# dohlee/chromoformer

Measured on AMD Instinct MI355X. Metric: genes/sec training (bsz=64, default config), higher is better.
Workload: dtype f32

## Files before the change

### chromoformer_amd/csrc/cf_attc2.h

```cpp
#pragma once
#include <type_traits>

namespace cf {

struct Attc2Args {
    const float* feats[kMaxRes];
    const uint8_t* mask[kMaxRes];
    long long mstride[kMaxRes];
    const float* pe[kMaxRes];
    const float* pet[kMaxRes];
    const float* wlp[kMaxRes];
    const float* vin[kMaxRes];
    float* p[kMaxRes];
    float* w[kMaxRes];
    float* vout[kMaxRes];
    int L[kMaxRes], Lpad[kMaxRes], LT[kMaxRes];
    int N, F;
    float scale, rscale;
    unsigned long long* tdbg;
    unsigned long long* tall;
};
#define CF_STAMP2(slot)                                                                                   \
    do {                                                                                                  \
        if (a.tdbg && stamp_wg == 0 && (threadIdx.x & 63) == 0)                                            \
// ... 9 lines not shown

__device__ __forceinline__ void frag_load_nn_rt(FragNN<4, 8>& f, const float* __restrict__ Bm, int ldb, int nchunks) {
    const int lane = threadIdx.x & 63, r = lane & 15, q = lane >> 4;
    f.bp = Bm + (size_t)(q * 4) * ldb + 4 * r;
    f.ldb = ldb;
#pragma unroll
    for (int c = 0; c < kRing - 1; ++c) frag_chunk_nn(f, c, min(c, nchunks - 1));
    __builtin_amdgcn_sched_barrier(0);
}
__device__ __forceinline__ void frag_mma_nn_rt(FragNN<4, 8>& f, const float* As, int lda, int nchunks, f32x4 (&acc)[4]) {
    const int lane = threadIdx.x & 63, r = lane & 15, q = lane >> 4;
    const float* ap = As + r * lda + q * 4;
    float4 a_nxt = *reinterpret_cast<const float4*>(ap);
    for (int c0 = 0; c0 < nchunks; c0 += kRing) {
#pragma unroll
        for (int u = 0; u < kRing; ++u) {
            const int c = c0 + u;
            if (c + kRing - 1 < nchunks) frag_chunk_nn(f, (u + kRing - 1) % kRing, c + kRing - 1);
            __builtin_amdgcn_sched_barrier(0);
            if (c < nchunks)
#pragma unroll
                for (int k = 0; k < 2; ++k) {
                    const float4 a = a_nxt;
                    a_nxt = *reinterpret_cast<const float4*>(ap + (c * 2 + k + 1) * 16);
                    const float av[4] = {a.x, a.y, a.z, a.w};
#pragma unroll
                    for (int i = 0; i < 4; ++i) {
                        const float* bv = reinterpret_cast<const float*>(&f.ring[u][k][i]);
#pragma unroll
                        for (int t = 0; t < 4; ++t) acc[t] = mfma4(av[i], bv[t], acc[t]);
                    }
                }
        }
    }
}

__host__ __device__ inline size_t attc2_scratch_floats(int L) { return (size_t)kTile * (attc2_lpad(L) + 4) + 2 * kTile * (kD + 4) + 2 * kTile * 8; }
__host__ __device__ inline size_t attc2_persist_bytes(int L, int F, int AG) {
    return (size_t)(kD * 8 + AG * L * F + 8) * sizeof(float) + (size_t)AG * attc2_lpad(L);
}
template <int AG>
__device__ __forceinline__ void attc2_stage(const float* feats, const uint8_t* mask, long long mstride, const float* wlp, int L, int Lpad, int F,
                                            const int n0, const int N, float* persist) {
    const int tid = threadIdx.x, w = __builtin_amdgcn_readfirstlane(tid >> 6);
    float* wlp_s = persist;
    float* feats_s = wlp_s + kD * 8;
    uint8_t* mk_s = reinterpret_cast<uint8_t*>(feats_s + AG * L * F + 8);
    const int nreg = min(AG, N - n0);
    const float* fg = feats + (size_t)n0 * L * F;
    const int nf = nreg * L * F;
    constexpr int NFL = AG == 8 ? 12 : AG == 4 ? 6 : AG == 2 ? 3 : 2;
    const bool f16b = ((L * F) & 3) == 0 && AG * L * F <= NFL * 4 * kAT && (reinterpret_cast<uintptr_t>(fg) & 15) == 0;
    if (f16b) {
        const int n4 = (AG * L * F) >> 2, last4 = (nf >> 2) - 1;
#pragma unroll
        for (int u = 0; u < NFL; ++u) {
            const int i = tid + u * kAT;
            typedef __attribute__((address_space(3))) void* lds_void;
            typedef const __attribute__((address_space(1))) void* glb_void;
            if (i < n4)
                __builtin_amdgcn_global_load_lds((glb_void)(fg + (size_t)min(i, last4) * 4), (lds_void)(feats_s + (size_t)(w * 64 + u * kAT) * 4), 16, 0, 0);
        }
    } else {
        for (int i = tid; i < AG * L * F; i += kAT) feats_s[i] = i < nf ? ldg(fg + i) : 0.f;
    }
    if (tid < 8) feats_s[AG * L * F + tid] = 0.f;
    static_assert(kD * 8 == 2 * kAT, "wlp staging assumes two entries per thread");
    wlp_s[tid] = (tid & 7) < F ? ldg(wlp + (tid >> 3) * F + (tid & 7)) : 0.f;
    wlp_s[tid + kAT] = (tid & 7) < F ? ldg(wlp + ((tid + kAT) >> 3) * F + (tid & 7)) : 0.f;
    const uint8_t* mg = mask + (size_t)n0 * mstride;
    const bool words = ((L | (int)mstride | (int)(reinterpret_cast<uintptr_t>(mask))) & 3) == 0;
    if (words) {
        const int LW = Lpad >> 2, lw = L >> 2;
        uint32_t* mk_w = reinterpret_cast<uint32_t*>(mk_s);
        for (int idx = tid; idx < AG * LW; idx += kAT) {
            const int sreg = idx / LW, jw = idx - sreg * LW;
            mk_w[idx] = (sreg < nreg && jw < lw) ? *(const CF_GLOBAL uint32_t*)(mg + (size_t)sreg * mstride + 4 * jw) : 0x01010101u;
        }
    } else {
        for (int s = 0; s < AG; ++s)
            for (int j = tid; j < Lpad; j += kAT) mk_s[s * Lpad + j] = (s < nreg && j < L) ? *(const CF_GLOBAL uint8_t*)(mg + (size_t)s * mstride + j) : (uint8_t)1;
    }
}
template <bool BWD, int AG, bool STAGED = false>
__device__ __forceinline__ void attc2_body(const Attc2Args& a, const int r, const int n0, const int N, float* scratch, float* persist,
                                           const int stamp_wg = -1) {
    constexpr int kAG = AG;
    const int tid = threadIdx.x;
    const int w = tid >> 6, lane = tid & 63, lr = lane & 15, lq = lane >> 4;
    const int L = a.L[r], Lpad = a.Lpad[r], LT = a.LT[r], F = a.F, LS = Lpad + 4;
    constexpr int LD = kD + 4, NW = kAT / 64;
    float* sc_s = scratch;
    float* vin_s = sc_s + kTile * LS;
    float* red_s = vin_s + kTile * LD;
    float* u_s = red_s + kTile * LD;
    float* w_s = u_s + kTile * 8;
    float* wlp_s = persist;
    float* feats_s = wlp_s + kD * 8;
    uint8_t* mk_s = reinterpret_cast<uint8_t*>(feats_s + kAG * L * F + 8);
    const int nreg = min(kAG, N - n0);

    CF_STAMP2(0);
    if (a.tall && tid == 0 && stamp_wg >= 0) a.tall[stamp_wg * 2] = __builtin_amdgcn_s_memtime();
    const int nblk = (L + 63) / 64;
    float* stat_s = red_s;
    static_assert(2 * kTile * 16 <= kTile * LD, "statistics fit in the K-split partial buffer");
    FragNN<4, 8> ft0;
    const float* fg = a.feats[r] + (size_t)n0 * L * F;
    const int nf = nreg * L * F;
    constexpr int NFL = AG == 8 ? 12 : AG == 4 ? 6 : AG == 2 ? 3 : 2;
    const bool f16b = ((L * F) & 3) == 0 && kAG * L * F <= NFL * 4 * kAT;
    float4 fv12[NFL];
    {
        const uint8_t* mg = a.mask[r] + (size_t)n0 * a.mstride[r];
        const bool words = ((L | (int)a.mstride[r] | (int)(reinterpret_cast<uintptr_t>(a.mask[r]))) & 3) == 0;
        const int LW = Lpad >> 2, lw = L >> 2;
        constexpr int MW = kAG >= 2 ? kAG / 2 : 1;
        float4 vv = make_float4(0.f, 0.f, 0.f, 0.f);
        {
            const int m = tid >> 5, c4 = tid & 31;
            if ((m >> 1) < nreg) vv = ldg4(a.vin[r] + (size_t)n0 * 256 + m * kD + c4 * 4);
        }
        const float wl0 = !STAGED && (tid & 7) < F ? ldg(a.wlp[r] + (tid >> 3) * F + (tid & 7)) : 0.f;
        const float wl1 = !STAGED && (tid & 7) < F ? ldg(a.wlp[r] + ((tid + kAT) >> 3) * F + (tid & 7)) : 0.f;
        uint32_t mwv[MW];
        if (!STAGED && words) {
#pragma unroll
            for (int k = 0; k < MW; ++k) {
                const int idx = tid + k * kAT, sreg = idx / LW, jw = idx - sreg * LW;
                mwv[k] = (idx < kAG * LW && sreg < nreg && jw < lw) ? *(const CF_GLOBAL uint32_t*)(mg + (size_t)sreg * a.mstride[r] + 4 * jw) : 0x01010101u;
            }
        }
        {
            if (!STAGED) {
                const float* fa = reinterpret_cast<const float*>(reinterpret_cast<uintptr_t>(fg) & ~(uintptr_t)15);
                const int last4 = f16b ? (nf >> 2) - 1 : max((nf >> 2) - 2, 0);
#pragma unroll
                for (int u = 0; u < NFL; ++u) fv12[u] = ldg4(fa + (size_t)min(tid + u * kAT, last4) * 4);
            }
            const float* bm_ = a.pet[r] + min(w, nblk - 1) * 64;
            ft0.bp = bm_ + (size_t)(lq * 4) * LT + 4 * lr;
            ft0.ldb = LT;
            frag_chunk_nn(ft0, 0, 0);
        }
        __builtin_amdgcn_sched_barrier(0);
        stat_s[tid] = tid < kTile * 16 ? 0.f : -INFINITY;
        if (tid < kTile) u_s[tid * 8 + 7] = 0.f;
        {
            const int m = tid >> 5;
            for (int j = L + (tid & 31); j < Lpad; j += 32) sc_s[m * LS + j] = 0.f;
        }
        *reinterpret_cast<float4*>(vin_s + (tid >> 5) * LD + (tid & 31) * 4) = vv;
        static_assert(kD * 8 == 2 * kAT, "wlp staging assumes two entries per thread");
        if (!STAGED) {
            wlp_s[tid] = wl0;
            wlp_s[tid + kAT] = wl1;
        }
        if (STAGED) {
        } else if (words) {
            uint32_t* mk_w = reinterpret_cast<uint32_t*>(mk_s);
#pragma unroll
            for (int k = 0; k < MW; ++k)
                if (tid + k * kAT < kAG * LW) mk_w[tid + k * kAT] = mwv[k];
        } else {
            for (int s = 0; s < kAG; ++s)
                for (int j = tid; j < Lpad; j += kAT)
                    mk_s[s * Lpad + j] = (s < nreg && j < L) ? *(const CF_GLOBAL uint8_t*)(mg + (size_t)s * a.mstride[r] + j) : (uint8_t)1;
        }
    }
    CF_STAMP2(10);
    __syncthreads();
    CF_STAMP2(1);
    float ub[32];
    if (w == NW - 1) {
        const float* wp_ = a.wlp[r] + (size_t)(lq * 4) * F + min(lr, F - 1);
#pragma unroll
        for (int st8 = 0; st8 < 8; ++st8)
#pragma unroll
            for (int i = 0; i < 4; ++i) ub[st8 * 4 + i] = ldg(wp_ + (size_t)(st8 * 16 + i) * F);
    }
    f32x4 acc2[2][4];
    zero_acc(acc2[0]);
    zero_acc(acc2[1]);
    {
        const float* ap = vin_s + lr * LD + lq * 4;
        auto products = [&](auto c_c) {
            constexpr int c = decltype(c_c)::value;
            if (w < nblk)
#pragma unroll
                for (int k = 0; k < 2; ++k) {
                    const float4 av4 = *reinterpret_cast<const float4*>(ap + (c * 2 + k) * 16);
                    const float av[4] = {av4.x, av4.y, av4.z, av4.w};
#pragma unroll
                    for (int i = 0; i < 4; ++i) {
                        const float* bv = reinterpret_cast<const float*>(&ft0.ring[c][k][i]);
#pragma unroll
                        for (int t = 0; t < 4; ++t) acc2[0][t] = mfma4(av[i], bv[t], acc2[0][t]);
                    }
                }
        };
        frag_chunk_nn(ft0, 1, 1);
        frag_chunk_nn(ft0, 2, 2);
        __builtin_amdgcn_sched_barrier(0);
        if (w == NW - 1) {
            f32x4 ua = {0.f, 0.f, 0.f, 0.f};
#pragma unroll
            for (int st8 = 0; st8 < 8; ++st8) {
                const float4 av = *reinterpret_cast<const float4*>(ap + st8 * 16);
                ua = mfma4(av.x, ub[st8 * 4], ua);
                ua = mfma4(av.y, ub[st8 * 4 + 1], ua);
                ua = mfma4(av.z, ub[st8 * 4 + 2], ua);
                ua = mfma4(av.w, ub[st8 * 4 + 3], ua);
            }
            if (lr < F)
#pragma unroll
                for (int ii = 0; ii < 4; ++ii) u_s[(lq * 4 + ii) * 8 + lr] = ua[ii];
        }
        __builtin_amdgcn_sched_barrier(0);
        products(std::integral_constant<int, 0>{});
        __builtin_amdgcn_sched_barrier(0);
        frag_chunk_nn(ft0, 3, 3);
        __builtin_amdgcn_sched_barrier(0);
        products(std::integral_constant<int, 1>{});
        products(std::integral_constant<int, 2>{});
        products(std::integral_constant<int, 3>{});
    }
    if (w + NW < nblk) {
        FragNN<4, 8> ft;
        frag_load_nn(ft, a.pet[r] + (w + NW) * 64, LT);
        frag_mma_nn(ft, vin_s, LD, acc2[1]);
    }
    CF_STAMP2(8);
    if (STAGED) {
    } else if (f16b) {
        const int n4 = (kAG * L * F) >> 2;
#pragma unroll
        for (int u = 0; u < NFL; ++u) {
            const int i = tid + u * kAT;
            if (i < n4) *reinterpret_cast<float4*>(feats_s + (size_t)i * 4) = fv12[u];
        }
        if (tid < 8) feats_s[kAG * L * F + tid] = 0.f;
    } else {
        for (int i = tid; i < kAG * L * F + 8; i += kAT) feats_s[i] = i < nf ? ldg(fg + i) : 0.f;
    }
    const int cg = w & 1, kh = w >> 1, kper = Lpad / 4;
    FragNN<4, 8> fp5;
    frag_load_nn_rt(fp5, a.pe[r] + (size_t)(kh * kper) * kD + cg * 64, kD, kper / 32);
    CF_STAMP2(9);
    __syncthreads();
    CF_STAMP2(2);
    float xs[2][4][4];
    float4 pv[2][4];
    float bstat[2][4];
#pragma unroll
    for (int bi = 0; bi < 2; ++bi) {
        const int jb = w + bi * NW;
        if (jb >= nblk) continue;
        const int j0 = jb * 64 + 4 * lr;
        if (BWD) {
#pragma unroll
            for (int ii = 0; ii < 4; ++ii) {
                const int m = lq * 4 + ii;
                pv[bi][ii] = make_float4(0.f, 0.f, 0.f, 0.f);
                if ((m >> 1) < nreg && (m >> 1) < kAG) {
                    const float* pg = a.p[r] + ((size_t)n0 * 2 + m) * L;
                    if (j0 + 3 < L && (L & 3) == 0) pv[bi][ii] = (CF_TRUNK_NT & 2) ? ldg4_nt(pg + j0) : ldg4(pg + j0);
                    else {
                        if (j0 < L) pv[bi][ii].x = ldg(pg + j0);
                        if (j0 + 1 < L) pv[bi][ii].y = ldg(pg + j0 + 1);
                        if (j0 + 2 < L) pv[bi][ii].z = ldg(pg + j0 + 2);
                        if (j0 + 3 < L) pv[bi][ii].w = ldg(pg + j0 + 3);
                    }
                }
            }
        }
#pragma unroll
        for (int sp = 0; sp < 2; ++sp) {
            const int s = lq * 2 + sp;
            if (s >= kAG) continue;
            float fv[4][8];
            if (j0 + 3 < L && F == 7) {
                const float4* fp4 = reinterpret_cast<const float4*>(feats_s + (size_t)(s * L + j0) * 7);
                float tmp[28];
#pragma unroll
                for (int k = 0; k < 7; ++k) {
                    const float4 t4 = fp4[k];
                    tmp[4 * k] = t4.x;
                    tmp[4 * k + 1] = t4.y;
                    tmp[4 * k + 2] = t4.z;
                    tmp[4 * k + 3] = t4.w;
                }
#pragma unroll
                for (int t = 0; t < 4; ++t)
#pragma unroll
                    for (int f = 0; f < 8; ++f) fv[t][f] = f < 7 ? tmp[t * 7 + f] : 0.f;
            } else {
#pragma unroll
                for (int t = 0; t < 4; ++t)
#pragma unroll
                    for (int f = 0; f < 8; ++f) fv[t][f] = (j0 + t < L && f < F) ? feats_s[(size_t)(s * L + j0 + t) * F + f] : 0.f;
            }
            const uint32_t mw = *reinterpret_cast<const uint32_t*>(mk_s + s * Lpad + j0);
#pragma unroll
            for (int hd = 0; hd < 2; ++hd) {
                const int ii = sp * 2 + hd, m = lq * 4 + ii;
                const float4 u0 = *reinterpret_cast<const float4*>(u_s + m * 8), u1 = *reinterpret_cast<const float4*>(u_s + m * 8 + 4);
                float bm = -INFINITY;
#pragma unroll
                for (int t = 0; t < 4; ++t) {
                    float x = acc2[bi][t][ii];
                    x = fmaf(fv[t][0], u0.x, x);
                    x = fmaf(fv[t][1], u0.y, x);
                    x = fmaf(fv[t][2], u0.z, x);
                    x = fmaf(fv[t][3], u0.w, x);
                    x = fmaf(fv[t][4], u1.x, x);
                    x = fmaf(fv[t][5], u1.y, x);
                    x = fmaf(fv[t][6], u1.z, x);
                    x = fmaf(fv[t][7], u1.w, x);
                    if (!BWD) {
                        x = x * a.rscale;
                        if ((mw >> (8 * t)) & 0xffu) x = kMaskFill;
                        if (j0 + t < L) bm = fmaxf(bm, x);
                    }
                    xs[bi][ii][t] = x;
                }
                float part;
                if (!BWD) {
                    bm = group16_max(bm);
                    part = 0.f;
#pragma unroll
                    for (int t = 0; t < 4; ++t) {
                        const float e = j0 + t < L ? __expf(xs[bi][ii][t] - bm) : 0.f;
                        xs[bi][ii][t] = e;
                        part += e;
                    }
                    bstat[bi][ii] = bm;
                } else {
                    const float4 p4 = pv[bi][ii];
                    part = (p4.x * xs[bi][ii][0] + p4.y * xs[bi][ii][1]) + (p4.z * xs[bi][ii][2] + p4.w * xs[bi][ii][3]);
                }
                part = group16_sum(part);
                if (lr == 0) {
                    stat_s[m * 16 + jb] = part;
                    if (!BWD) stat_s[kTile * 16 + m * 16 + jb] = bm;
                }
            }
        }
    }
    __syncthreads();
    CF_STAMP2(3);
#pragma unroll
    for (int ii = 0; ii < 4; ++ii) {
        const int m = lq * 4 + ii, s = m >> 1;
        if (s >= kAG || w >= nblk) continue;
        const bool present = s < nreg;
        float fac[2] = {0.f, 0.f}, dot = 0.f;
        const float bsum = stat_s[m * 16 + lr];
        if (!BWD) {
            const float bmax = stat_s[kTile * 16 + m * 16 + lr];
            const float mx = group16_max(bmax);
            const float z = group16_sum(bsum * __expf(bmax - mx));
            const float rz = 1.0f / z;
#pragma unroll
            for (int bi = 0; bi < 2; ++bi) fac[bi] = (w + bi * NW < nblk) ? __expf(bstat[bi][ii] - mx) * rz : 0.f;
        } else {
            dot = group16_sum(bsum);
        }
#pragma unroll
        for (int bi = 0; bi < 2; ++bi) {
            const int jb = w + bi * NW;
            if (jb >= nblk) continue;
            const int j0 = jb * 64 + 4 * lr;
            float4 o;
            if (!BWD) {
                o = make_float4(xs[bi][ii][0] * fac[bi], xs[bi][ii][1] * fac[bi], xs[bi][ii][2] * fac[bi], xs[bi][ii][3] * fac[bi]);
                if (present) {
                    float* pg = a.p[r] + ((size_t)n0 * 2 + m) * L;
                    if (j0 + 3 < L && (L & 3) == 0) {
                        if (CF_TRUNK_NT & 1) stg4_nt(pg + j0, o);
                        else stg4(pg + j0, o);
                    }
                    else {
                        if (j0 < L) stg(pg + j0, o.x);
                        if (j0 + 1 < L) stg(pg + j0 + 1, o.y);
                        if (j0 + 2 < L) stg(pg + j0 + 2, o.z);
                        if (j0 + 3 < L) stg(pg + j0 + 3, o.w);
                    }
                }
            } else {
                const uint32_t mw = *reinterpret_cast<const uint32_t*>(mk_s + s * Lpad + j0);
                const float4 p4 = pv[bi][ii];
                o.x = (mw & 0xffu) ? 0.f : p4.x * (xs[bi][ii][0] - dot) * a.rscale;
                o.y = (mw & 0xff00u) ? 0.f : p4.y * (xs[bi][ii][1] - dot) * a.rscale;
// ... 148 lines not shown
```

### chromoformer_amd/csrc/cf_trunk.h

```cpp
#pragma once

namespace cf {

constexpr int kMaxPairLayers = 4;

struct CentreLayerDev {
    const float *wq_t, *wk, *wv_t, *wo_t, *bo, *g1, *be1, *w1_t, *b1, *w2_t, *b2, *g2, *be2;
    const float *wq, *wk_t, *wv, *wo, *w1, *w2;
    float *q, *qt, *p, *w, *xbar, *a, *xh1, *rs1, *y1, *hdn, *xh2, *rs2, *out, *xin;
    float *dt2, *dpre1, *dt1, *da, *dxbar, *dqt, *du, *dq, *dx, *partial;
};
struct TrunkResDev {
    CentreLayerDev E, P[kMaxPairLayers];
    const float *pe, *pe2, *pet2;
    const float *wlp_e, *wlp_p;
    const float *lin_p_t, *lin_p;
    float *ex0, *featc, *xp0, *dxp0, *edout, *rx0, *drx0;
    float *lp_part_e, *lp_part_p;
    int L, Lpad, LT, pad_;
};
struct TrunkArgs {
    const TrunkResDev* tab;
    const float* pfeats[kMaxRes];
    const uint8_t* pmask[kMaxRes];
    long long pmstride[kMaxRes];
    const float* cfeats[kMaxRes];
    const uint8_t* cmask[kMaxRes];
    long long cmstride[kMaxRes];
    const float* dhin;
    int B, S, T, F, n_res, pair_layers, save;
    float scale, rscale;
    const RetileUnit* rt_units;
    const float* rt_params;
    float* rt_tiled;
    float* rt_tiledT;
    int rt_n;
    RecordArgs rec;
    int* adv_cursor;
    const LpJob* lp_jobs;
    const WgTile* rd_tiles;
    int rd_n, rd_batch;
    AdamFuse rd_opt;
    unsigned long long* tdbg;
};

template <class T>
__device__ __forceinline__ T ldc(const T* p) {
    static_assert(sizeof(T) == 8 || sizeof(T) == 4, "pointer or int fields");
    if constexpr (sizeof(T) == 8) {
        const unsigned long long v = *(const __attribute__((address_space(4))) unsigned long long*)p;
        return __builtin_bit_cast(T, v);
    } else {
        const unsigned v = *(const __attribute__((address_space(4))) unsigned*)p;
        return __builtin_bit_cast(T, v);
    }
}
#define TF(field) ldc(&R->field)

__host__ __device__ inline size_t trunk_scratch_floats(int L, int dff_max) {
    const size_t chain = (size_t)3 * kTile * (kD + 4) + (size_t)kTile * ((dff_max > 256 ? dff_max : 256) + 4);
    const size_t att = attc2_scratch_floats(L);
    return (chain > att ? chain : att) + 4;
}
__host__ __device__ inline size_t trunk_smem(int L, int F, int dff_max) {
    const size_t two = trunk_scratch_floats(L, dff_max) * sizeof(float) + attc2_persist_bytes(L, F, kAGMax);
    const size_t one = attc1_smem(L, F);
    const size_t rt = (size_t)(kAT / 64) * 16 * 20 * sizeof(float);
    const size_t lp = (size_t)80 * (kD + 8) * sizeof(float);
    size_t m = two > one ? two : one;
    m = m > rt ? m : rt;
    return m > lp ? m : lp;
}

#ifndef CF_STAMP_Y
#define CF_STAMP_Y 0
#endif
#define CF_PHASE static __device__ __forceinline__

struct TrunkCtx {
    const TrunkResDev* R;
    const float* feats;
    const uint8_t* mask;
    long long mstride;
    int g, S, T, F, save;
    float scale, rscale;
};
__device__ __forceinline__ void launder(TrunkCtx& c, float*& smem, float*& persist) {
    asm volatile("" : "+s"(c.R), "+s"(c.feats), "+s"(c.mask), "+s"(c.mstride), "+s"(c.g), "+s"(c.S), "+s"(c.T), "+s"(c.F), "+s"(c.save),
                 "+s"(c.scale), "+s"(c.rscale));
    typedef __attribute__((address_space(3))) float* lds_ptr;
    unsigned a = (unsigned)(uintptr_t)(lds_ptr)smem, b = (unsigned)(uintptr_t)(lds_ptr)persist;
    asm volatile("" : "+s"(a), "+s"(b));
    smem = (float*)(lds_ptr)(uintptr_t)a;
    persist = (float*)(lds_ptr)(uintptr_t)b;
}
__device__ __forceinline__ void trunk_attc_args(Attc2Args& at, const TrunkCtx& c, const float* wlp, const float* vin, float* p, float* w, float* vout,
                                                int N) {
    const TrunkResDev* R = c.R;
    at.feats[0] = c.feats;
    at.mask[0] = c.mask;
    at.mstride[0] = c.mstride;
    at.pe[0] = TF(pe2);
    at.pet[0] = TF(pet2);
    at.wlp[0] = wlp;
    at.vin[0] = vin;
    at.p[0] = p;
    at.w[0] = w;
    at.vout[0] = vout;
    at.L[0] = TF(L);
    at.Lpad[0] = TF(Lpad);
    at.LT[0] = TF(LT);
    at.N = N;
    at.F = c.F;
    at.scale = c.scale;
    at.rscale = c.rscale;
    at.tdbg = nullptr;
    at.tall = nullptr;
}
#define CF_CHAIN_TILES(scratch)                                                                       \
    float (*xs)[kD + 4] = reinterpret_cast<float (*)[kD + 4]>(scratch);                               \
    float (*as_)[kD + 4] = reinterpret_cast<float (*)[kD + 4]>((scratch) + kTile * (kD + 4));         \
    float (*ts)[kD + 4] = reinterpret_cast<float (*)[kD + 4]>((scratch) + 2 * kTile * (kD + 4));      \
    float* wide_raw = (scratch) + 3 * kTile * (kD + 4);                                               \
    (void)xs, (void)as_, (void)ts, (void)wide_raw

}
#include "cf_trunk_e.h"
namespace cf {

template <bool BWD>
CF_PHASE void trunk_attc1_e(TrunkCtx c, float* smem) {
    const TrunkResDev* R = c.R;
    Attc2Args at;
    if (!BWD) trunk_attc_args(at, c, TF(wlp_e), TF(E.qt), TF(E.p), TF(E.w), TF(E.xbar), c.g + 1);
    else trunk_attc_args(at, c, TF(wlp_e), TF(E.dxbar), TF(E.p), TF(E.du), TF(E.dqt), c.g + 1);
    attc1_body<BWD>(at, 0, c.g, smem);
}
__device__ __forceinline__ void trunk_post_args(PostArgs& po, const CentreLayerDev* P, int save) {
    po.ain[0] = ldc(&P->xbar);
    po.wv[0] = ldc(&P->wv_t);
    po.wo[0] = ldc(&P->wo_t);
    po.bo[0] = ldc(&P->bo);
    po.g1[0] = ldc(&P->g1);
    po.be1[0] = ldc(&P->be1);
    po.w1[0] = ldc(&P->w1_t);
    po.b1[0] = ldc(&P->b1);
    po.w2[0] = ldc(&P->w2_t);
    po.b2[0] = ldc(&P->b2);
    po.g2[0] = ldc(&P->g2);
    po.be2[0] = ldc(&P->be2);
    po.a_out[0] = ldc(&P->a);
    po.xh1[0] = ldc(&P->xh1);
    po.rs1[0] = ldc(&P->rs1);
    po.y1[0] = ldc(&P->y1);
    po.hdn[0] = ldc(&P->hdn);
    po.xh2[0] = ldc(&P->xh2);
    po.rs2[0] = ldc(&P->rs2);
    po.save = save;
    po.lin_w[0] = nullptr;
    po.nq_wq[0] = nullptr;
}
CF_PHASE void trunk_qchain_p0(TrunkCtx c, float* smem) {
    const TrunkResDev* R = c.R;
    CF_CHAIN_TILES(smem);
    const CentreLayerDev* P0 = &R->P[0];
    QChainArgs q;
    q.x[0] = TF(xp0);
    q.xmap = RowMap{c.S, 1, 0, 0};
    q.wq[0] = ldc(&P0->wq_t);
    q.wk[0] = ldc(&P0->wk);
    q.q[0] = ldc(&P0->q);
    q.qt[0] = ldc(&P0->qt);
    q.xcopy[0] = ldc(&P0->xin);
    q.N = c.g * c.S + c.S;
    qchain_fwd_body<kAT / 64>(q, 0, c.g * c.S, xs, as_);
}
template <bool BWD, bool STAGED>
CF_PHASE void trunk_attc2_p(TrunkCtx c, int l, float* scratch, float* persist) {
    const TrunkResDev* R = c.R;
    const CentreLayerDev* P = &R->P[l];
    const int row0 = c.g * c.S, NB = row0 + c.S;
    Attc2Args at;
    if (!BWD) trunk_attc_args(at, c, TF(wlp_p), ldc(&P->qt), ldc(&P->p), ldc(&P->w), ldc(&P->xbar), NB);
    else trunk_attc_args(at, c, TF(wlp_p), ldc(&P->dxbar), ldc(&P->p), ldc(&P->du), ldc(&P->dqt), NB);
    attc2_body<BWD, kAGMax, STAGED>(at, 0, row0, NB, scratch, persist);
}
CF_PHASE void trunk_stage_p(TrunkCtx c, float* persist) {
    const TrunkResDev* R = c.R;
    attc2_stage<kAGMax>(c.feats, c.mask, c.mstride, TF(wlp_p), TF(L), TF(Lpad), c.F, c.g * c.S, c.g * c.S + c.S, persist);
}
template <int DFF>
CF_PHASE void trunk_post_p(TrunkCtx c, int l, int n_layers, float* smem) {
    const TrunkResDev* R = c.R;
    const CentreLayerDev* P = &R->P[l];
    const bool last = l + 1 == n_layers;
    const int S = c.S, row0 = c.g * S, NB = row0 + S;
    CF_CHAIN_TILES(smem);
    PostArgs po;
    trunk_post_args(po, P, c.save);
    po.x[0] = l == 0 ? (const float*)TF(xp0) : (const float*)ldc(&R->P[l > 0 ? l - 1 : 0].out);
    po.xmap = l == 0 ? RowMap{S, 1, 0, 0} : identity_map();
    po.out[0] = last ? TF(rx0) : ldc(&P->out);
    po.omap = last ? RowMap{S, c.T, 1, 1} : identity_map();
    po.N = NB;
    if (!last) {
        const CentreLayerDev* Pn = &R->P[l + 1];
        po.nq_wq[0] = ldc(&Pn->wq_t);
        po.nq_wk[0] = ldc(&Pn->wk);
        po.nq_q[0] = ldc(&Pn->q);
        po.nq_qt[0] = ldc(&Pn->qt);
    }
    post_fwd_body<true, 128, DFF, kAT / 64>(po, 0, row0, NB, xs, as_, ts, reinterpret_cast<float (*)[PostFwdLds<DFF>::HW + 4]>(wide_raw));
}

template <int DFF_E, int DFF_P, int PL>
__global__ __launch_bounds__(kAT) void k_trunk_fwd(TrunkArgs a) {
    extern __shared__ __attribute__((aligned(16))) float smem[];
    constexpr int NWV = kAT / 64;
    if ((int)blockIdx.y >= a.n_res) {
        float (*tp)[16][20] = reinterpret_cast<float (*)[16][20]>(smem);
        for (int u = blockIdx.x; u < a.rt_n; u += gridDim.x) {
            retile_unit_lds<NWV>(a.rt_params, a.rt_tiled, a.rt_tiledT, a.rt_units[u], tp);
            __syncthreads();
        }
        return;
    }
    if (a.adv_cursor && blockIdx.x == 0 && blockIdx.y == 0 && threadIdx.x == 0 && a.adv_cursor[0] < a.adv_cursor[1]) a.adv_cursor[0] += 1;
    const int r = a.n_res - 1 - (int)blockIdx.y;
    const TrunkResDev* R = a.tab + r;
    constexpr int DFF_MAX = DFF_E > DFF_P ? DFF_E : DFF_P;
    float* sm = smem;
    float* persist = smem + trunk_scratch_floats(TF(L), DFF_MAX);
    TrunkCtx c{R, a.pfeats[r], a.pmask[r], a.pmstride[r], (int)blockIdx.x, a.S, a.T, a.F, a.save, a.scale, a.rscale};
    int stamp_i = 0;
    if (a.tdbg && blockIdx.x == 0 && blockIdx.y == CF_STAMP_Y && threadIdx.x == 0) a.tdbg[stamp_i++] = __builtin_amdgcn_s_memtime();
#define CF_NEXT_PHASE                                                                                     \
    __syncthreads();                                                                                      \
    if (a.tdbg && blockIdx.x == 0 && blockIdx.y == CF_STAMP_Y && threadIdx.x == 0) a.tdbg[stamp_i++] = __builtin_amdgcn_s_memtime(); \
    launder(c, sm, persist)
    {
        TrunkCtx cs{R, a.cfeats[r], a.cmask[r], a.cmstride[r], (int)blockIdx.x, a.S, a.T, a.F, a.save, a.scale, a.rscale};
        trunk_stage_p(cs, persist);
        launder(c, sm, persist);
    }
    trunk_e_front(c, sm);
    CF_NEXT_PHASE;
    trunk_attc1_e<false>(c, sm);
    CF_NEXT_PHASE;
    trunk_e_post_fwd<DFF_E>(c, sm);
    c.feats = a.cfeats[r];
    c.mask = a.cmask[r];
    c.mstride = a.cmstride[r];
    CF_NEXT_PHASE;
    trunk_qchain_p0(c, sm);
    asm volatile("s_waitcnt vmcnt(0)" ::: "memory");
    CF_NEXT_PHASE;
    trunk_attc2_p<false, true>(c, 0, sm, persist);
    CF_NEXT_PHASE;
    trunk_post_p<DFF_P>(c, 0, PL, sm);
#pragma unroll
    for (int l = 1; l < PL; ++l) {
        CF_NEXT_PHASE;
        trunk_attc2_p<false, true>(c, l, sm, persist);
        CF_NEXT_PHASE;
        trunk_post_p<DFF_P>(c, l, PL, sm);
    }
    CF_NEXT_PHASE;
}

__device__ __forceinline__ void trunk_post_bwd_args(PostBwdArgs& pb, const CentreLayerDev* P) {
    pb.xh2[0] = ldc(&P->xh2);
    pb.rs2[0] = ldc(&P->rs2);
    pb.g2[0] = ldc(&P->g2);
    pb.hdn[0] = ldc(&P->hdn);
    pb.w2[0] = ldc(&P->w2);
    pb.w1[0] = ldc(&P->w1);
    pb.xh1[0] = ldc(&P->xh1);
    pb.rs1[0] = ldc(&P->rs1);
    pb.g1[0] = ldc(&P->g1);
    pb.wo[0] = ldc(&P->wo);
    pb.wv[0] = ldc(&P->wv);
    pb.dt2[0] = ldc(&P->dt2);
    pb.dpre1[0] = ldc(&P->dpre1);
    pb.dt1[0] = ldc(&P->dt1);
    pb.da[0] = ldc(&P->da);
    pb.dxbar[0] = ldc(&P->dxbar);
    pb.partial[0] = ldc(&P->partial);
}
#define CF_BWD_TILES(DFF)                                                                                       \
    constexpr int WW_ = (DFF) > 128 ? (DFF) : 128;                                                              \
    float (*wide)[WW_ + 4] = reinterpret_cast<float (*)[WW_ + 4]>(wide_raw)
template <int DFF>
CF_PHASE void trunk_post_bwd_p(TrunkCtx c, int l, int n_layers, float* smem) {
    const TrunkResDev* R = c.R;
    const CentreLayerDev* P = &R->P[l];
    const bool last = l + 1 == n_layers;
    const int S = c.S, row0 = c.g * S, NB = row0 + S;
    CF_CHAIN_TILES(smem);
    CF_BWD_TILES(DFF);
    PostBwdArgs pb;
    trunk_post_bwd_args(pb, P);
    pb.dout[0] = last ? (const float*)TF(drx0) : (const float*)ldc(&R->P[last ? l : l + 1].dx);
    pb.dmap = last ? RowMap{S, c.T, 1, 1} : identity_map();
    pb.N = NB;
    post_bwd_body<true, 128, DFF, kAT / 64>(pb, 0, row0, NB, c.g, xs, as_, ts, wide);
}
CF_PHASE void trunk_qchain_bwd(TrunkCtx c, const CentreLayerDev* P, int row0, int NB, float* smem) {
    float (*ds)[256 + 4] = reinterpret_cast<float (*)[256 + 4]>(smem);
    float (*qs)[kD + 4] = reinterpret_cast<float (*)[kD + 4]>(smem + kTile * (256 + 4));
    QBwdArgs qb;
    qb.dqt[0] = ldc(&P->dqt);
    qb.dres[0] = ldc(&P->dt1);
    qb.wk[0] = ldc(&P->wk_t);
    qb.wq[0] = ldc(&P->wq);
    qb.dq[0] = ldc(&P->dq);
    qb.dx[0] = ldc(&P->dx);
    qb.N = NB;
    (void)c;
    qchain_bwd_body<kAT / 64>(qb, 0, row0, ds, qs);
}
CF_PHASE void trunk_join(TrunkCtx c, const float* dhin, int r, int n_res, float* smem) {
    const TrunkResDev* R = c.R;
    const int g = c.g, S = c.S, tid = threadIdx.x;
    float* xk = smem;
    float* red = smem + kD;
    if (tid < kD) {
        const float* dxp = ldc(&R->P[0].dx) + (size_t)g * S * kD + tid;
        float s = 0.f;
        for (int i = 0; i < S; ++i) s += ldg(dxp + (size_t)i * kD);
        xk[tid] = s;
        stg(TF(dxp0) + (size_t)g * kD + tid, s);
    }
    __syncthreads();
    {
        const int col = tid & (kD - 1), kw = (tid >> 7) * 32;
        const float* w = TF(lin_p) + (size_t)kw * kD + col;
        float acc = 0.f;
#pragma unroll
        for (int k = 0; k < 2; ++k)
#pragma unroll
// ... 130 lines not shown
```

### chromoformer_amd/csrc/cf_trunk_e.h

```cpp
#pragma once

namespace cf {

static_assert(kAT == kMvT, "the one-row products of cf_valu_mv.h are laid out for the trunk's workgroup size");

constexpr int kEvX = 0;
constexpr int kEvB = 128;
constexpr int kEvA = 384;
constexpr int kEvT = 512;
constexpr int kEvH = 640;
constexpr int kEvX2 = 896;
constexpr int kEvW = 1024;
constexpr int kEvW2 = 2048;
constexpr int kEvP = 3072;
constexpr int kEvEnd = kEvP + 16 * 256;

CF_PHASE void trunk_e_front(TrunkCtx c, float* smem) {
    const TrunkResDev* R = c.R;
    const int g = c.g, tid = threadIdx.x;
    float* xs = smem + kEvX;
    float* qs = smem + kEvA;
    float* part = smem + kEvP;
    NtW<kD, kD> wq;
    nt_request(wq, TF(E.wq_t));
// ... 35 lines not shown
    const TrunkResDev* R = c.R;
    const int g = c.g, tid = threadIdx.x, w = tid >> 6, lane = tid & 63;
    const bool save = c.save != 0;
    float* xs = smem + kEvX;
    float* xb = smem + kEvB;
    float* as_ = smem + kEvA;
    float* ts = smem + kEvT;
    float* hs = smem + kEvH;
    float* y1w = smem + kEvW + w * kD;
    float* ow = smem + kEvW2 + w * kD;
    static_assert(DFF == 128 || DFF == 256, "hidden width of the Embedding layer");
    NtW<kD, kD> wv, wo;
    nt_request(wv, TF(E.wv_t));
    float rx = 0.f, rb = 0.f;
    if (tid < kD) rx = ldg(TF(ex0) + (size_t)g * kD + tid);
    if (tid < 2 * kD) rb = ldg(TF(E.xbar) + (size_t)g * 2 * kD + tid);
    nt_request(wo, TF(E.wo_t));
    const int n = nt_row<kD, kD>(0);
    const float g1a = ldg(TF(E.g1) + lane), g1b = ldg(TF(E.g1) + lane + 64), b1a = ldg(TF(E.be1) + lane), b1b = ldg(TF(E.be1) + lane + 64);
    const float g2a = ldg(TF(E.g2) + lane), g2b = ldg(TF(E.g2) + lane + 64), b2a = ldg(TF(E.be2) + lane), b2b = ldg(TF(E.be2) + lane + 64);
    const float bo = ldg(TF(E.bo) + n), b2 = ldg(TF(E.b2) + n);
    __builtin_amdgcn_sched_barrier(0);
    if (tid < kD) xs[tid] = rx;
    if (tid < 2 * kD) xb[tid] = rb;
    __syncthreads();
    {
        float a[1];
        nt_dot(wv, xb + (n >> 6) * kD, a);
        if (nt_writer()) {
            as_[n] = a[0];
            if (save) stg(TF(E.a) + (size_t)g * kD + n, a[0]);
        }
    }
    NtW<DFF, kD> w1;
    nt_request(w1, TF(E.w1_t));
    __builtin_amdgcn_sched_barrier(0);
    __syncthreads();
    {
        float t[1];
        nt_dot(wo, as_, t);
        if (nt_writer()) ts[n] = t[0] + bo + xs[n];
    }
    NtW<kD, DFF> w2;
    nt_request(w2, TF(E.w2_t));
    float b1[NtW<DFF, kD>::TW];
#pragma unroll
    for (int t = 0; t < NtW<DFF, kD>::TW; ++t) b1[t] = ldg(TF(E.b1) + nt_row<DFF, kD>(t));
    __builtin_amdgcn_sched_barrier(0);
    __syncthreads();
    {
        const LnRow o = ln_row_fwd(ts[lane], ts[lane + 64], g1a, g1b, b1a, b1b);
        y1w[lane] = o.y0;
        y1w[lane + 64] = o.y1;
        if (w == 0 && save) {
            stg(TF(E.xh1) + (size_t)g * kD + lane, o.x0);
            stg(TF(E.xh1) + (size_t)g * kD + lane + 64, o.x1);
            stg(TF(E.y1) + (size_t)g * kD + lane, o.y0);
            stg(TF(E.y1) + (size_t)g * kD + lane + 64, o.y1);
            if (lane == 0) stg(TF(E.rs1) + g, o.rstd);
        }
    }
    __builtin_amdgcn_wave_barrier();
    {
        float v[NtW<DFF, kD>::TW];
        nt_dot(w1, y1w, v);
        if (nt_writer())
#pragma unroll
            for (int t = 0; t < NtW<DFF, kD>::TW; ++t) {
                const int j = nt_row<DFF, kD>(t);
                const float hv = fmaxf(v[t] + b1[t], 0.f);
                hs[j] = hv;
                if (save) stg(TF(E.hdn) + (size_t)g * DFF + j, hv);
            }
    }
    NtW<kD, kD> wl;
    nt_request(wl, TF(lin_p_t));
    __builtin_amdgcn_sched_barrier(0);
    __syncthreads();
    {
        float t[1];
        nt_dot(w2, hs, t);
        if (nt_writer()) ts[n] = t[0] + b2 + y1w[n];
    }
    __syncthreads();
    {
        const LnRow o = ln_row_fwd(ts[lane], ts[lane + 64], g2a, g2b, b2a, b2b);
        ow[lane] = o.y0;
        ow[lane + 64] = o.y1;
        if (w == 0) {
            if (save) {
                stg(TF(E.xh2) + (size_t)g * kD + lane, o.x0);
                stg(TF(E.xh2) + (size_t)g * kD + lane + 64, o.x1);
                if (lane == 0) stg(TF(E.rs2) + g, o.rstd);
            }
            float* rx0 = TF(rx0) + (size_t)g * c.T * kD;
            stg(rx0 + lane, o.y0);
            stg(rx0 + lane + 64, o.y1);
        }
    }
    __builtin_amdgcn_wave_barrier();
    {
        float v[1];
        nt_dot(wl, ow, v);
        if (nt_writer()) stg(TF(xp0) + (size_t)g * kD + n, v[0]);
    }
}

template <int DFF>
CF_PHASE void trunk_e_post_bwd(TrunkCtx c, float* smem) {
    const TrunkResDev* R = c.R;
    const int g = c.g, tid = threadIdx.x, w = tid >> 6, lane = tid & 63;
    float* dys = smem + kEvA;
    float* das = smem + kEvA;
    float* hs = smem + kEvH;
    float* dt2w = smem + kEvW + w * kD;
    float* dt1w = smem + kEvW2 + w * kD;
    float* part = smem + kEvP;
    float* prow = TF(E.partial) + (size_t)g * post_partial_width(DFF);
    TrW<kD, DFF> w2;
    tr_request(w2, TF(E.w2));
    const float d0 = ldg(TF(edout) + (size_t)g * kD + lane), d1 = ldg(TF(edout) + (size_t)g * kD + lane + 64);
    const float x20 = ldg(TF(E.xh2) + (size_t)g * kD + lane), x21 = ldg(TF(E.xh2) + (size_t)g * kD + lane + 64);
    const float x10 = ldg(TF(E.xh1) + (size_t)g * kD + lane), x11 = ldg(TF(E.xh1) + (size_t)g * kD + lane + 64);
    const float rs2 = ldg(TF(E.rs2) + g), rs1 = ldg(TF(E.rs1) + g);
    const float g2a = ldg(TF(E.g2) + lane), g2b = ldg(TF(E.g2) + lane + 64), g1a = ldg(TF(E.g1) + lane), g1b = ldg(TF(E.g1) + lane + 64);
    float hv = 0.f;
    if (tid < DFF) hv = ldg(TF(E.hdn) + (size_t)g * DFF + tid);
    TrW<DFF, kD> w1;
    tr_request(w1, TF(E.w1));
    __builtin_amdgcn_sched_barrier(0);
    float t20, t21;
    ln_row_bwd(d0, d1, g2a, g2b, x20, x21, rs2, t20, t21);
    dt2w[lane] = t20;
    dt2w[lane + 64] = t21;
    if (w == 0) {
        stg(TF(E.dt2) + (size_t)g * kD + lane, t20);
        stg(TF(E.dt2) + (size_t)g * kD + lane + 64, t21);
        stg(prow + lane, d0 * x20);
        stg(prow + lane + 64, d1 * x21);
        stg(prow + 128 + lane, d0);
        stg(prow + 128 + lane + 64, d1);
        stg(prow + 256 + lane, t20);
        stg(prow + 256 + lane + 64, t21);
    }
    __builtin_amdgcn_wave_barrier();
    tr_partial(w2, dt2w, part);
    TrW<kD, kD> wo;
    tr_request(wo, TF(E.wo));
    __builtin_amdgcn_sched_barrier(0);
    __syncthreads();
    if (tid < DFF) {
        const float s = tr_sum<DFF>(part, 0, TrW<kD, DFF>::NG, tid);
        const float dp = hv > 0.f ? s : 0.f;
        hs[tid] = dp;
        stg(TF(E.dpre1) + (size_t)g * DFF + tid, dp);
        stg(prow + 384 + tid, dp);
    }
    __syncthreads();
    tr_partial(w1, hs, part);
    __syncthreads();
    if (tid < kD) dys[tid] = dt2w[tid] + tr_sum<kD>(part, 0, TrW<DFF, kD>::NG, tid);
    TrW<kD, kD> wv;
    tr_request(wv, TF(E.wv));
    __builtin_amdgcn_sched_barrier(0);
    __syncthreads();
    {
        const float y0 = dys[lane], y1 = dys[lane + 64];
        float t10, t11;
        ln_row_bwd(y0, y1, g1a, g1b, x10, x11, rs1, t10, t11);
        dt1w[lane] = t10;
        dt1w[lane + 64] = t11;
        if (w == 0) {
            stg(TF(E.dt1) + (size_t)g * kD + lane, t10);
            stg(TF(E.dt1) + (size_t)g * kD + lane + 64, t11);
            stg(prow + 384 + DFF + lane, y0 * x10);
            stg(prow + 384 + DFF + lane + 64, y1 * x11);
            stg(prow + 512 + DFF + lane, y0);
            stg(prow + 512 + DFF + lane + 64, y1);
            stg(prow + 640 + DFF + lane, t10);
            stg(prow + 640 + DFF + lane + 64, t11);
        }
    }
    __builtin_amdgcn_wave_barrier();
    tr_partial(wo, dt1w, part);
    __syncthreads();
    if (tid < kD) {
        const float s = tr_sum<kD>(part, 0, TrW<kD, kD>::NG, tid);
// ... 45 lines not shown
```

Measured before the change: 130,800.

## Fuse layer-0 query chain into embedding post phase and exploit shared query

Removes the separate qchain phase (and one grid-wide phase barrier) for the first pair-layer by computing the query projection and its key-projected form inside the embedding post phase, using the fact that every region row of a gene shares the same input row. The attention score phase for layer 0 then computes a single shared query-key product per gene with scalar FMA chains instead of per-row MFMA tiles. This cuts redundant work and synchronisation, at the cost of more registers for preloaded weights and scalar VALU dot products, plus redundant stores of the replicated query rows.

```diff
diff --git a/chromoformer_amd/csrc/cf_attc2.h b/chromoformer_amd/csrc/cf_attc2.h
--- a/chromoformer_amd/csrc/cf_attc2.h
+++ b/chromoformer_amd/csrc/cf_attc2.h
@@ -115,9 +115,10 @@
             for (int j = tid; j < Lpad; j += kAT) mk_s[s * Lpad + j] = (s < nreg && j < L) ? *(const CF_GLOBAL uint8_t*)(mg + (size_t)s * mstride + j) : (uint8_t)1;
     }
 }
-template <bool BWD, int AG, bool STAGED = false>
+template <bool BWD, int AG, bool STAGED = false, bool SHARED_Q = false>
 __device__ __forceinline__ void attc2_body(const Attc2Args& a, const int r, const int n0, const int N, float* scratch, float* persist,
                                            const int stamp_wg = -1) {
+    static_assert(!SHARED_Q || !BWD, "the shared-query variant is a forward variant");
     constexpr int kAG = AG;
     const int tid = threadIdx.x;
     const int w = tid >> 6, lane = tid & 63, lr = lane & 15, lq = lane >> 4;
@@ -144,6 +145,19 @@
     constexpr int NFL = AG == 8 ? 12 : AG == 4 ? 6 : AG == 2 ? 3 : 2;
     const bool f16b = ((L * F) & 3) == 0 && kAG * L * F <= NFL * 4 * kAT;
     float4 fv12[NFL];
+    float tb[4][32];
+    float* th_s = sc_s;
+    auto tb_request = [&](auto c_c) {
+        constexpr int c = decltype(c_c)::value;
+        const float* tp_ = a.pet[r] + tid;
+        if (tid < nblk * 64)
+#pragma unroll
+            for (int k2 = 0; k2 < 2; ++k2)
+#pragma unroll
+                for (int i = 0; i < 4; ++i)
+#pragma unroll
+                    for (int q = 0; q < 4; ++q) tb[c][k2 * 16 + i * 4 + q] = ldg(tp_ + (size_t)((c * 2 + k2) * 16 + q * 4 + i) * LT);
+    };
     {
         const uint8_t* mg = a.mask[r] + (size_t)n0 * a.mstride[r];
         const bool words = ((L | (int)a.mstride[r] | (int)(reinterpret_cast<uintptr_t>(a.mask[r]))) & 3) == 0;
@@ -171,10 +185,14 @@
 #pragma unroll
                 for (int u = 0; u < NFL; ++u) fv12[u] = ldg4(fa + (size_t)min(tid + u * kAT, last4) * 4);
             }
-            const float* bm_ = a.pet[r] + min(w, nblk - 1) * 64;
-            ft0.bp = bm_ + (size_t)(lq * 4) * LT + 4 * lr;
-            ft0.ldb = LT;
-            frag_chunk_nn(ft0, 0, 0);
+            if constexpr (SHARED_Q) {
+                tb_request(std::integral_constant<int, 0>{});
+            } else {
+                const float* bm_ = a.pet[r] + min(w, nblk - 1) * 64;
+                ft0.bp = bm_ + (size_t)(lq * 4) * LT + 4 * lr;
+                ft0.ldb = LT;
+                frag_chunk_nn(ft0, 0, 0);
+            }
         }
         __builtin_amdgcn_sched_barrier(0);
         stat_s[tid] = tid < kTile * 16 ? 0.f : -INFINITY;
@@ -215,25 +233,34 @@
     f32x4 acc2[2][4];
     zero_acc(acc2[0]);
     zero_acc(acc2[1]);
-    {
+    if constexpr (SHARED_Q) {
+        float t0 = 0.f, t1 = 0.f;
+        auto chains = [&](auto c_c) {
+            constexpr int c = decltype(c_c)::value;
+            if (tid < nblk * 64)
+#pragma unroll
+                for (int k2 = 0; k2 < 2; ++k2) {
+                    float v0[16], v1[16];
+#pragma unroll
+                    for (int q = 0; q < 4; ++q) {
+                        const float4 a0 = *reinterpret_cast<const float4*>(vin_s + (c * 2 + k2) * 16 + q * 4);
+                        const float4 a1 = *reinterpret_cast<const float4*>(vin_s + LD + (c * 2 + k2) * 16 + q * 4);
+                        v0[q * 4] = a0.x, v0[q * 4 + 1] = a0.y, v0[q * 4 + 2] = a0.z, v0[q * 4 + 3] = a0.w;
+                        v1[q * 4] = a1.x, v1[q * 4 + 1] = a1.y, v1[q * 4 + 2] = a1.z, v1[q * 4 + 3] = a1.w;
+                    }
+#pragma unroll
+                    for (int i = 0; i < 4; ++i)
+#pragma unroll
+                        for (int q = 0; q < 4; ++q) {
+                            const float b = tb[c][k2 * 16 + i * 4 + q];
+                            t0 = fmaf(v0[q * 4 + i], b, t0);
+                            t1 = fmaf(v1[q * 4 + i], b, t1);
+                        }
+                }
+        };
         const float* ap = vin_s + lr * LD + lq * 4;
-        auto products = [&](auto c_c) {
-            constexpr int c = decltype(c_c)::value;
-            if (w < nblk)
-#pragma unroll
-                for (int k = 0; k < 2; ++k) {
-                    const float4 av4 = *reinterpret_cast<const float4*>(ap + (c * 2 + k) * 16);
-                    const float av[4] = {av4.x, av4.y, av4.z, av4.w};
-#pragma unroll
-                    for (int i = 0; i < 4; ++i) {
-                        const float* bv = reinterpret_cast<const float*>(&ft0.ring[c][k][i]);
-#pragma unroll
-                        for (int t = 0; t < 4; ++t) acc2[0][t] = mfma4(av[i], bv[t], acc2[0][t]);
-                    }
-                }
-        };
-        frag_chunk_nn(ft0, 1, 1);
-        frag_chunk_nn(ft0, 2, 2);
+        tb_request(std::integral_constant<int, 1>{});
+        tb_request(std::integral_constant<int, 2>{});
         __builtin_amdgcn_sched_barrier(0);
         if (w == NW - 1) {
             f32x4 ua = {0.f, 0.f, 0.f, 0.f};
@@ -250,6 +277,68 @@
                 for (int ii = 0; ii < 4; ++ii) u_s[(lq * 4 + ii) * 8 + lr] = ua[ii];
         }
         __builtin_amdgcn_sched_barrier(0);
+        chains(std::integral_constant<int, 0>{});
+        __builtin_amdgcn_sched_barrier(0);
+        tb_request(std::integral_constant<int, 3>{});
+        __builtin_amdgcn_sched_barrier(0);
+        chains(std::integral_constant<int, 1>{});
+        chains(std::integral_constant<int, 2>{});
+        chains(std::integral_constant<int, 3>{});
+        if (tid < nblk * 64) {
+            th_s[tid] = t0;
+            th_s[LS + tid] = t1;
+        }
+        if (tid + kAT < nblk * 64) {
+            const float* tq = a.pet[r] + tid + kAT;
+            float s0 = 0.f, s1 = 0.f;
+            for (int kb = 0; kb < kD / 16; ++kb)
+#pragma unroll
+                for (int i = 0; i < 4; ++i)
+#pragma unroll
+                    for (int q = 0; q < 4; ++q) {
+                        const int k = kb * 16 + q * 4 + i;
+                        const float b = ldg(tq + (size_t)k * LT);
+                        s0 = fmaf(vin_s[k], b, s0);
+                        s1 = fmaf(vin_s[LD + k], b, s1);
+                    }
+            th_s[tid + kAT] = s0;
+            th_s[LS + tid + kAT] = s1;
+        }
+    } else {
+        const float* ap = vin_s + lr * LD + lq * 4;
+        auto products = [&](auto c_c) {
+            constexpr int c = decltype(c_c)::value;
+            if (w < nblk)
+#pragma unroll
+                for (int k = 0; k < 2; ++k) {
+                    const float4 av4 = *reinterpret_cast<const float4*>(ap + (c * 2 + k) * 16);
+                    const float av[4] = {av4.x, av4.y, av4.z, av4.w};
+#pragma unroll
+                    for (int i = 0; i < 4; ++i) {
+                        const float* bv = reinterpret_cast<const float*>(&ft0.ring[c][k][i]);
+#pragma unroll
+                        for (int t = 0; t < 4; ++t) acc2[0][t] = mfma4(av[i], bv[t], acc2[0][t]);
+                    }
+                }
+        };
+        frag_chunk_nn(ft0, 1, 1);
+        frag_chunk_nn(ft0, 2, 2);
+        __builtin_amdgcn_sched_barrier(0);
+        if (w == NW - 1) {
+            f32x4 ua = {0.f, 0.f, 0.f, 0.f};
+#pragma unroll
+            for (int st8 = 0; st8 < 8; ++st8) {
+                const float4 av = *reinterpret_cast<const float4*>(ap + st8 * 16);
+                ua = mfma4(av.x, ub[st8 * 4], ua);
+                ua = mfma4(av.y, ub[st8 * 4 + 1], ua);
+                ua = mfma4(av.z, ub[st8 * 4 + 2], ua);
+                ua = mfma4(av.w, ub[st8 * 4 + 3], ua);
+            }
+            if (lr < F)
+#pragma unroll
+                for (int ii = 0; ii < 4; ++ii) u_s[(lq * 4 + ii) * 8 + lr] = ua[ii];
+        }
+        __builtin_amdgcn_sched_barrier(0);
         products(std::integral_constant<int, 0>{});
         __builtin_amdgcn_sched_barrier(0);
         frag_chunk_nn(ft0, 3, 3);
@@ -258,7 +347,7 @@
         products(std::integral_constant<int, 2>{});
         products(std::integral_constant<int, 3>{});
     }
-    if (w + NW < nblk) {
+    if (!SHARED_Q && w + NW < nblk) {
         FragNN<4, 8> ft;
         frag_load_nn(ft, a.pet[r] + (w + NW) * 64, LT);
         frag_mma_nn(ft, vin_s, LD, acc2[1]);
@@ -339,9 +428,14 @@
                 const int ii = sp * 2 + hd, m = lq * 4 + ii;
                 const float4 u0 = *reinterpret_cast<const float4*>(u_s + m * 8), u1 = *reinterpret_cast<const float4*>(u_s + m * 8 + 4);
                 float bm = -INFINITY;
+                float tv[4] = {0.f, 0.f, 0.f, 0.f};
+                if constexpr (SHARED_Q) {
+                    const float4 t4 = *reinterpret_cast<const float4*>(th_s + hd * LS + j0);
+                    tv[0] = t4.x, tv[1] = t4.y, tv[2] = t4.z, tv[3] = t4.w;
+                }
 #pragma unroll
                 for (int t = 0; t < 4; ++t) {
-                    float x = acc2[bi][t][ii];
+                    float x = SHARED_Q ? tv[t] : acc2[bi][t][ii];
                     x = fmaf(fv[t][0], u0.x, x);
                     x = fmaf(fv[t][1], u0.y, x);
                     x = fmaf(fv[t][2], u0.z, x);
diff --git a/chromoformer_amd/csrc/cf_trunk.h b/chromoformer_amd/csrc/cf_trunk.h
--- a/chromoformer_amd/csrc/cf_trunk.h
+++ b/chromoformer_amd/csrc/cf_trunk.h
@@ -76,6 +76,9 @@
 #define CF_STAMP_Y 0
 #endif
 #define CF_PHASE static __device__ __forceinline__
+#ifndef CF_SHARED_Q
+#define CF_SHARED_Q 1
+#endif
 
 struct TrunkCtx {
     const TrunkResDev* R;
@@ -160,22 +163,7 @@
     po.lin_w[0] = nullptr;
     po.nq_wq[0] = nullptr;
 }
-CF_PHASE void trunk_qchain_p0(TrunkCtx c, float* smem) {
-    const TrunkResDev* R = c.R;
-    CF_CHAIN_TILES(smem);
-    const CentreLayerDev* P0 = &R->P[0];
-    QChainArgs q;
-    q.x[0] = TF(xp0);
-    q.xmap = RowMap{c.S, 1, 0, 0};
-    q.wq[0] = ldc(&P0->wq_t);
-    q.wk[0] = ldc(&P0->wk);
-    q.q[0] = ldc(&P0->q);
-    q.qt[0] = ldc(&P0->qt);
-    q.xcopy[0] = ldc(&P0->xin);
-    q.N = c.g * c.S + c.S;
-    qchain_fwd_body<kAT / 64>(q, 0, c.g * c.S, xs, as_);
-}
-template <bool BWD, bool STAGED>
+template <bool BWD, bool STAGED, bool SHARED_Q = false>
 CF_PHASE void trunk_attc2_p(TrunkCtx c, int l, float* scratch, float* persist) {
     const TrunkResDev* R = c.R;
     const CentreLayerDev* P = &R->P[l];
@@ -183,7 +171,7 @@
     Attc2Args at;
     if (!BWD) trunk_attc_args(at, c, TF(wlp_p), ldc(&P->qt), ldc(&P->p), ldc(&P->w), ldc(&P->xbar), NB);
     else trunk_attc_args(at, c, TF(wlp_p), ldc(&P->dxbar), ldc(&P->p), ldc(&P->du), ldc(&P->dqt), NB);
-    attc2_body<BWD, kAGMax, STAGED>(at, 0, row0, NB, scratch, persist);
+    attc2_body<BWD, kAGMax, STAGED, SHARED_Q>(at, 0, row0, NB, scratch, persist);
 }
 CF_PHASE void trunk_stage_p(TrunkCtx c, float* persist) {
     const TrunkResDev* R = c.R;
@@ -251,11 +239,9 @@
     c.feats = a.cfeats[r];
     c.mask = a.cmask[r];
     c.mstride = a.cmstride[r];
-    CF_NEXT_PHASE;
-    trunk_qchain_p0(c, sm);
     asm volatile("s_waitcnt vmcnt(0)" ::: "memory");
     CF_NEXT_PHASE;
-    trunk_attc2_p<false, true>(c, 0, sm, persist);
+    trunk_attc2_p<false, true, CF_SHARED_Q != 0>(c, 0, sm, persist);
     CF_NEXT_PHASE;
     trunk_post_p<DFF_P>(c, 0, PL, sm);
 #pragma unroll
diff --git a/chromoformer_amd/csrc/cf_trunk_e.h b/chromoformer_amd/csrc/cf_trunk_e.h
--- a/chromoformer_amd/csrc/cf_trunk_e.h
+++ b/chromoformer_amd/csrc/cf_trunk_e.h
@@ -141,6 +141,20 @@
         nt_dot(w2, hs, t);
         if (nt_writer()) ts[n] = t[0] + b2 + y1w[n];
     }
+    float4 wqp[kD / 16][4];
+    if (tid < kD) {
+        const float* wp = TF(P[0].wq_t) + (size_t)(tid >> 4) * 16 * kD + (tid & 15) * 4;
+#pragma unroll
+        for (int kb = 0; kb < kD / 16; ++kb)
+#pragma unroll
+            for (int q = 0; q < 4; ++q) wqp[kb][q] = ldg4(wp + kb * 256 + q * 64);
+    }
+    float wkp[kD / 2];
+    const float* wkp_ = TF(P[0].wk) + (size_t)(((tid >> 7) & 1) * (kD / 2)) * kD + (tid & (kD - 1));
+    if (tid < 2 * kD)
+#pragma unroll
+        for (int k = 0; k < kD / 4; ++k) wkp[k] = ldg(wkp_ + (size_t)k * kD);
+    __builtin_amdgcn_sched_barrier(0);
     __syncthreads();
     {
         const LnRow o = ln_row_fwd(ts[lane], ts[lane + 64], g2a, g2b, b2a, b2b);
@@ -161,7 +175,57 @@
     {
         float v[1];
         nt_dot(wl, ow, v);
-        if (nt_writer()) stg(TF(xp0) + (size_t)g * kD + n, v[0]);
+        if (nt_writer()) {
+            xs[n] = v[0];
+            stg(TF(xp0) + (size_t)g * kD + n, v[0]);
+        }
+    }
+    if (tid < 2 * kD)
+#pragma unroll
+        for (int k = kD / 4; k < kD / 2; ++k) wkp[k] = ldg(wkp_ + (size_t)k * kD);
+    __builtin_amdgcn_sched_barrier(0);
+    __syncthreads();
+    const int S = c.S;
+    const size_t row0 = (size_t)g * S;
+    if (tid < kD) {
+        float q = 0.f;
+#pragma unroll
+        for (int kb = 0; kb < kD / 16; ++kb) {
+            float x[16];
+#pragma unroll
+            for (int j = 0; j < 4; ++j) {
+                const float4 x4 = *reinterpret_cast<const float4*>(xs + kb * 16 + j * 4);
+                x[j * 4] = x4.x, x[j * 4 + 1] = x4.y, x[j * 4 + 2] = x4.z, x[j * 4 + 3] = x4.w;
+            }
+#pragma unroll
+            for (int i = 0; i < 4; ++i)
+#pragma unroll
+                for (int j = 0; j < 4; ++j) q = fmaf(x[j * 4 + i], reinterpret_cast<const float*>(&wqp[kb][j])[i], q);
+        }
+        as_[tid] = q;
+        for (int s = 0; s < S; ++s) stg(TF(P[0].q) + (row0 + s) * kD + tid, q);
+    } else {
+        for (int i = tid - kD; i < S * (kD / 4); i += kMvT - kD)
+            stg4(TF(P[0].xin) + (row0 + (i >> 5)) * kD + (i & 31) * 4, *reinterpret_cast<const float4*>(xs + (i & 31) * 4));
+    }
+    __syncthreads();
+    if (tid < 2 * kD) {
+        const float* qh = as_ + (tid >> 7) * (kD / 2);
+        float v = 0.f;
+#pragma unroll
+        for (int kb = 0; kb < kD / 32; ++kb) {
+            float x[16];
+#pragma unroll
+            for (int j = 0; j < 4; ++j) {
+                const float4 x4 = *reinterpret_cast<const float4*>(qh + kb * 16 + j * 4);
+                x[j * 4] = x4.x, x[j * 4 + 1] = x4.y, x[j * 4 + 2] = x4.z, x[j * 4 + 3] = x4.w;
+            }
+#pragma unroll
+            for (int i = 0; i < 4; ++i)
+#pragma unroll
+                for (int j = 0; j < 4; ++j) v = fmaf(x[j * 4 + i], wkp[kb * 16 + j * 4 + i], v);
+        }
+        for (int s = 0; s < S; ++s) stg(TF(P[0].qt) + (row0 + s) * 2 * kD + tid, v);
     }
 }
 
```

Result: no change. 131,700 (median of 6 runs) (+0.7%).
